# Adamtaranto/frisk

Measured on AMD Instinct MI355X. Metric: windows/sec (k=1..8, w=5kb, s=1kb), higher is better.
Workload: dtype u8/u4 counts + f64 scores

## Files before the change

### frisk_amd/csrc/profile_kernels.h

```cpp
#pragma once
#include "frisk_device.h"

#define FRISK_PROF_NT 1024

struct ProfRange {
    const uint32_t* __restrict__ codes;
    const uint32_t* __restrict__ inv;
    const uint32_t* __restrict__ low;
    int64_t p0, p1;
    int mask_host;
    __device__ int64_t w_first() const { return p0 >> 5; }
    __device__ int64_t w_end() const { return (p1 + 31) >> 5; }
    __device__ void chunk(int64_t i, int64_t chunk_words, int64_t& wb, int64_t& we) const {
        wb = w_first() + i * chunk_words;
        we = wb + chunk_words;
        if (we > w_end()) we = w_end();
    }
};

__device__ __forceinline__ uint32_t topbits(int64_t k) {
    k = k < 0 ? 0 : (k > 32 ? 32 : k);
    return uint32_t(0xFFFFFFFF00000000ull >> k);
}

struct ProfWord {
    uint32_t inr;
    uint32_t other;
    uint64_t V;
    uint64_t NP;
    uint64_t lo64, hi64;
};

__device__ __forceinline__ ProfWord load_word(const ProfRange& r, int64_t wq) {
    const int64_t base = wq << 5;
    const uint32_t i0 = r.inv[wq], i1 = r.inv[wq + 1], l0 = r.low[wq], l1 = r.low[wq + 1];
    const uint32_t c0 = r.codes[2 * wq], c1 = r.codes[2 * wq + 1], c2 = r.codes[2 * wq + 2];
    const uint32_t e0 = i0 | (r.mask_host ? l0 : 0u), e1 = i1 | (r.mask_host ? l1 : 0u);
    ProfWord W;
    W.inr = topbits(r.p1 - base) & ~topbits(r.p0 - base);
    W.other = i0 | l0;
    W.V = ~((uint64_t(e0) << 32) | e1);
    W.NP = ~((uint64_t(i0 & l0) << 32) | (i1 & l1));
    W.lo64 = (uint64_t(c0) << 32) | c1;
    W.hi64 = (uint64_t(c1) << 32) | c2;
    return W;
}

template <bool K8>
__device__ __forceinline__ uint64_t run_starts(uint64_t M, int k) {
    uint64_t F = M;
    if (K8) { F &= F << 1; F &= F << 2; F &= F << 4; }
    else for (int s = 1; s < k; ++s) F &= M << s;
    return F;
}

template <int BITS>
__device__ __forceinline__ uint32_t code_at(const ProfWord& W, int j) {
    return uint32_t((j < 16 ? W.lo64 : W.hi64) >> (64 - BITS - 2 * (j & 15))) & ((1u << BITS) - 1u);
}

template <int BITS>
__device__ __forceinline__ void add_runs(const ProfWord& W, uint32_t todo, int kmin, int kmax, unsigned long long* __restrict__ raw) {
    while (todo) {
        const int j = __clz(int(todo));
        todo &= ~(0x80000000u >> j);
        int run = __clzll((long long)(~(W.V << j)));
        run = run < kmax ? run : kmax;
        if (run >= kmin) atomicAdd(&raw[table_offset(kmin, run) + (code_at<BITS>(W, j) >> (BITS - 2 * run))], 1ull);
    }
}

__device__ __forceinline__ unsigned long long wave_sum(unsigned long long v) {
    for (int o = 32; o > 0; o >>= 1) v += __shfl_down(v, o);
    return v;
}

struct ProfScalars {
    unsigned long long tot = 0, kpos = 0, nn = 0;
    template <bool K8>
    __device__ __forceinline__ void add(const ProfWord& W, int kmax) {
        const uint64_t G = run_starts<K8>(W.NP, kmax);
        const uint32_t real = uint32_t(W.NP >> 32) & W.inr;
        tot += __popc(real);
        nn += __popc(real & W.other);
        kpos += __popc(uint32_t(G >> 32) & W.inr);
    }
    __device__ __forceinline__ void flush(unsigned long long* __restrict__ tail) {
        tot = wave_sum(tot);
        kpos = wave_sum(kpos);
        nn = wave_sum(nn);
        if ((threadIdx.x & 63) == 0) {
            if (tot) atomicAdd(&tail[0], tot);
            if (kpos) atomicAdd(&tail[1], kpos);
            if (nn) atomicAdd(&tail[2], nn);
        }
    }
};

__device__ __forceinline__ void clear_table(uint32_t* hist, uint32_t nwords) {
    for (uint32_t b = threadIdx.x; b < nwords / 4; b += blockDim.x) reinterpret_cast<uint4*>(hist)[b] = make_uint4(0, 0, 0, 0);
    if (nwords < 4) for (uint32_t b = threadIdx.x; b < nwords; b += blockDim.x) hist[b] = 0;
}
__device__ __forceinline__ void flush_table32(const uint32_t* hist, uint32_t nbins, unsigned long long* __restrict__ dst) {
    for (uint32_t b = threadIdx.x; b < nbins; b += blockDim.x) {
        const uint32_t v = hist[b];
        if (v) atomicAdd(&dst[b], (unsigned long long)v);
    }
}

struct HalfTable {
    uint32_t* hist;
    uint32_t nbins, halfbit, mine;
    int shK;
    __device__ __forceinline__ HalfTable(uint32_t* hist_, int kmax, int halves, int half)
        : hist(hist_), nbins((1u << (2 * kmax)) / uint32_t(halves)), halfbit(halves == 2 ? nbins : 0u), mine(half ? halfbit : 0u),
          shK(16 - 2 * kmax) {}
    __device__ __forceinline__ void operator()(uint32_t c16) const {
        const uint32_t code = c16 >> shK;
        if ((code & halfbit) == mine) atomicAdd(&hist[code & (nbins - 1)], 1u);
    }
};

template <bool K8, class Full>
__device__ __forceinline__ unsigned long long walk_words(const ProfRange& r, int64_t wb, int64_t we, int kmin, int kmax, bool rest,
                                                         unsigned long long* __restrict__ raw, int nprof, const Full& full) {
    ProfScalars S;
    unsigned long long counted = 0;
    for (int64_t wq = wb + threadIdx.x; wq < we; wq += blockDim.x) {
        const ProfWord W = load_word(r, wq);
        const uint64_t F = run_starts<K8>(W.V, kmax);
        const uint32_t fullm = uint32_t(F >> 32) & W.inr;
#pragma unroll
        for (int j = 0; j < 32; ++j)
            if (fullm & (0x80000000u >> j)) full(code_at<16>(W, j));
        if (rest) {
            counted += uint32_t(__popc(fullm));
            add_runs<16>(W, uint32_t(W.V >> 32) & ~uint32_t(F >> 32) & W.inr, kmin, kmax, raw);
            S.add<K8>(W, kmax);
        }
    }
    if (rest) S.flush(raw + nprof);
    return counted;
}

__global__ __launch_bounds__(FRISK_PROF_NT) void profile_add_kernel(const uint32_t* __restrict__ codes,
                                                                     const uint32_t* __restrict__ inv,
                                                                     const uint32_t* __restrict__ low, int64_t p0, int64_t p1,
                                                                     int kmin, int kmax, int mask_host, int nprof,
                                                                     int halves, int64_t chunk_words,
                                                                     unsigned long long* __restrict__ raw) {
    extern __shared__ __attribute__((aligned(16))) uint32_t hist[];
    const int half = int(blockIdx.x) % halves;
    const HalfTable table(hist, kmax, halves, half);
    clear_table(hist, table.nbins);
    __syncthreads();
    const ProfRange r{codes, inv, low, p0, p1, mask_host};
    int64_t wb, we;
    r.chunk(int64_t(blockIdx.x) / halves, chunk_words, wb, we);
    walk_words<false>(r, wb, we, kmin, kmax, half == 0, raw, nprof, table);
    __syncthreads();
    flush_table32(hist, table.nbins, raw + table_offset(kmin, kmax) + uint32_t(half) * table.nbins);
}

__global__ __launch_bounds__(FRISK_PROF_NT) void profile_add16_kernel(const uint32_t* __restrict__ codes,
                                                                       const uint32_t* __restrict__ inv,
                                                                       const uint32_t* __restrict__ low, int64_t p0, int64_t p1,
                                                                       int kmin, int mask_host, int nprof, int64_t chunk_words,
                                                                       unsigned long long* __restrict__ raw) {
    constexpr int K = 8;
    constexpr uint32_t NW = (1u << (2 * K)) / 2;
    extern __shared__ __attribute__((aligned(16))) uint32_t hist[];
    __shared__ unsigned long long red[2];
    clear_table(hist, NW);
    if (threadIdx.x < 2) red[threadIdx.x] = 0ull;
    __syncthreads();
    const ProfRange r{codes, inv, low, p0, p1, mask_host};
    int64_t wb, we;
    r.chunk(int64_t(blockIdx.x), chunk_words, wb, we);
    const int64_t offK = table_offset(kmin, K);
    const unsigned long long counted = wave_sum(walk_words<true>(r, wb, we, kmin, K, true, raw, nprof, [&](uint32_t code) {
        atomicAdd(&hist[code >> 1], 1u << ((code & 1u) * 16u));
    }));
    if ((threadIdx.x & 63) == 0 && counted) atomicAdd(&red[0], counted);
    __syncthreads();
    {
        unsigned long long sum = 0;
        for (uint32_t b = threadIdx.x; b < NW; b += blockDim.x) { const uint32_t v = hist[b]; sum += (v & 0xFFFFu) + (v >> 16); }
        sum = wave_sum(sum);
        if ((threadIdx.x & 63) == 0 && sum) atomicAdd(&red[1], sum);
    }
    __syncthreads();
    if (red[0] == red[1]) {
        for (uint32_t b = threadIdx.x; b < NW; b += blockDim.x) {
            const uint32_t v = hist[b];
            if (v & 0xFFFFu) atomicAdd(&raw[offK + 2u * b], (unsigned long long)(v & 0xFFFFu));
            if (v >> 16) atomicAdd(&raw[offK + 2u * b + 1u], (unsigned long long)(v >> 16));
        }
        return;
    }
    for (int half = 0; half < 2; ++half) {
        __syncthreads();
        clear_table(hist, NW);
        __syncthreads();
        walk_words<true>(r, wb, we, kmin, K, false, raw, nprof, HalfTable(hist, K, 2, half));
        __syncthreads();
        flush_table32(hist, NW, raw + offK + uint32_t(half) * NW);
    }
}

__global__ __launch_bounds__(256) void profile_add_big_kernel(const uint32_t* __restrict__ codes, const uint32_t* __restrict__ inv,
                                                               const uint32_t* __restrict__ low, int64_t p0, int64_t p1, int kmin,
                                                               int kmax, int mask_host, int nprof,
                                                               unsigned long long* __restrict__ raw) {
    const ProfRange r{codes, inv, low, p0, p1, mask_host};
    ProfScalars S;
    for (int64_t wq = r.w_first() + int64_t(blockIdx.x) * blockDim.x + threadIdx.x; wq < r.w_end(); wq += int64_t(gridDim.x) * blockDim.x) {
        const ProfWord W = load_word(r, wq);
        add_runs<24>(W, uint32_t(W.V >> 32) & W.inr, kmin, kmax, raw);
        S.add<false>(W, kmax);
    }
    S.flush(raw + nprof);
}

__global__ __launch_bounds__(256) void marginalize_kernel(int64_t* __restrict__ cnt, int kmin, int x) {
    const int64_t q = int64_t(blockIdx.x) * blockDim.x + threadIdx.x;
    if (q >= (int64_t(1) << (2 * x))) return;
    const int64_t* up = cnt + table_offset(kmin, x + 1) + 4 * q;
    cnt[table_offset(kmin, x) + q] += up[0] + up[1] + up[2] + up[3];
}

__global__ __launch_bounds__(1024) void marginalize_low_kernel(int64_t* __restrict__ cnt, int kmin, int x_hi) {
    for (int x = x_hi; x >= kmin; --x) {
        const int64_t n = int64_t(1) << (2 * x);
        int64_t* dst = cnt + table_offset(kmin, x);
        const int64_t* up = cnt + table_offset(kmin, x + 1);
        for (int64_t q = threadIdx.x; q < n; q += blockDim.x) dst[q] += up[4 * q] + up[4 * q + 1] + up[4 * q + 2] + up[4 * q + 3];
        __threadfence_block();
        __syncthreads();
    }
}

__global__ __launch_bounds__(256) void symmetrize_kernel(const int64_t* __restrict__ fwd, int64_t* __restrict__ sym,
                                                          int kmin, int kmax) {
    const int64_t t = int64_t(blockIdx.x) * blockDim.x + threadIdx.x;
    for (int x = kmin; x <= kmax; ++x) {
        const int64_t off = table_offset(kmin, x), n = int64_t(1) << (2 * x);
        if (t >= off && t < off + n) {
            const uint32_t c = uint32_t(t - off);
            sym[t] = fwd[t] + fwd[off + revcomp_code(c, x)];
        }
    }
}

#pragma clang fp contract(off)
__global__ __launch_bounds__(1024) void profile_meta_kernel(const int64_t* __restrict__ cnt, const int64_t* __restrict__ raw_tail,
                                                             int kmin, int kmax, int64_t* __restrict__ meta) {
    __shared__ long long part[16];
    const int64_t n = int64_t(1) << (2 * kmax);
    const int64_t* top = cnt + table_offset(kmin, kmax);
    long long s = 0;
    for (int64_t i = threadIdx.x; i < n; i += blockDim.x) s += top[i];
    for (int o = 32; o > 0; o >>= 1) s += __shfl_down(s, o);
    if ((threadIdx.x & 63) == 0) part[threadIdx.x >> 6] = s;
    __syncthreads();
    if (threadIdx.x == 0) {
        long long counted = 0;
        for (int w = 0; w < int(blockDim.x >> 6); ++w) counted += part[w];
        meta[0] = raw_tail[0];
        meta[1] = raw_tail[1] - counted;
        meta[2] = raw_tail[2];
    }
}

__global__ __launch_bounds__(256) void genome_ivom_kernel(const int64_t* __restrict__ sym, int kmin, int kmax,
                                                           const int64_t* __restrict__ meta, double* __restrict__ ig) {
    const int64_t k = int64_t(blockIdx.x) * blockDim.x + threadIdx.x;
    if (k >= (int64_t(1) << (2 * kmax))) return;
    const int64_t genome_space = meta[0] - meta[2];
    unsigned long long W = 0;
    double I = 0.0;
    bool bad = false;
    for (int x = kmin; x <= kmax; ++x) {
        const int64_t c = sym[table_offset(kmin, x) + (k >> (2 * (kmax - x)))];
        const unsigned long long wt = (unsigned long long)c << (2 * x);
        W += wt;
        const int64_t D = (genome_space - (x - 1)) * 2;
        if (W == 0 || D == 0) { bad = true; break; }
        const double p = double(c) / double(D);
        const double a = double(wt) / double(W);
        I = (x == kmin) ? a * p : a * p + ((1.0 - a) * I);
    }
    ig[k] = bad ? __longlong_as_double(0x7FF8000000000000LL) : I;
}
```

Before: 68.18 million.

## Repack k=8 shared histogram by top bit and add all-full wave fast path

Changes the packed 16-bit shared histogram so the top code bit picks the upper or lower half-word instead of the lowest bit. The index becomes a plain shift-and-mask of the unmasked code window, and the half select uses a bitfield extract. It also adds a wave-uniform fast path: when every lane's word is fully covered by k-runs, the per-j bit tests and the add_runs loop are skipped. The flush maps the two half-words to the bins b and NW+b. This adds inline asm and a wave vote, and correctness depends on the new index mapping matching the raw table layout.

```diff
diff --git a/frisk_amd/csrc/profile_kernels.h b/frisk_amd/csrc/profile_kernels.h
--- a/frisk_amd/csrc/profile_kernels.h
+++ b/frisk_amd/csrc/profile_kernels.h
@@ -1,5 +1,8 @@
 #pragma once
 #include "frisk_device.h"
+#ifdef FRISK_PROFILE_DEBUG
+#include <cassert>
+#endif
 
 #define FRISK_PROF_NT 1024
 
@@ -59,6 +62,10 @@
     return uint32_t((j < 16 ? W.lo64 : W.hi64) >> (64 - BITS - 2 * (j & 15))) & ((1u << BITS) - 1u);
 }
 
+__device__ __forceinline__ uint32_t code4_at(const ProfWord& W, int j) {
+    return uint32_t((j < 16 ? W.lo64 : W.hi64) >> (46 - 2 * (j & 15)));
+}
+
 template <int BITS>
 __device__ __forceinline__ void add_runs(const ProfWord& W, uint32_t todo, int kmin, int kmax, unsigned long long* __restrict__ raw) {
     while (todo) {
@@ -115,8 +122,8 @@
     __device__ __forceinline__ HalfTable(uint32_t* hist_, int kmax, int halves, int half)
         : hist(hist_), nbins((1u << (2 * kmax)) / uint32_t(halves)), halfbit(halves == 2 ? nbins : 0u), mine(half ? halfbit : 0u),
           shK(16 - 2 * kmax) {}
-    __device__ __forceinline__ void operator()(uint32_t c16) const {
-        const uint32_t code = c16 >> shK;
+    __device__ __forceinline__ void operator()(uint32_t c4) const {
+        const uint32_t code = ((c4 >> 2) & 0xFFFFu) >> shK;
         if ((code & halfbit) == mine) atomicAdd(&hist[code & (nbins - 1)], 1u);
     }
 };
@@ -130,9 +137,21 @@
         const ProfWord W = load_word(r, wq);
         const uint64_t F = run_starts<K8>(W.V, kmax);
         const uint32_t fullm = uint32_t(F >> 32) & W.inr;
+        if (__all(fullm == 0xFFFFFFFFu)) {
+#pragma unroll
+            for (int j = 0; j < 32; ++j) full(code4_at(W, j));
+            if (rest) {
+#ifdef FRISK_PROFILE_DEBUG
+                assert((uint32_t(W.V >> 32) & ~uint32_t(F >> 32) & W.inr) == 0u);
+#endif
+                counted += 32u;
+                S.add<K8>(W, kmax);
+            }
+            continue;
+        }
 #pragma unroll
         for (int j = 0; j < 32; ++j)
-            if (fullm & (0x80000000u >> j)) full(code_at<16>(W, j));
+            if (fullm & (0x80000000u >> j)) full(code4_at(W, j));
         if (rest) {
             counted += uint32_t(__popc(fullm));
             add_runs<16>(W, uint32_t(W.V >> 32) & ~uint32_t(F >> 32) & W.inr, kmin, kmax, raw);
@@ -178,8 +197,10 @@
     int64_t wb, we;
     r.chunk(int64_t(blockIdx.x), chunk_words, wb, we);
     const int64_t offK = table_offset(kmin, K);
-    const unsigned long long counted = wave_sum(walk_words<true>(r, wb, we, kmin, K, true, raw, nprof, [&](uint32_t code) {
-        atomicAdd(&hist[code >> 1], 1u << ((code & 1u) * 16u));
+    const unsigned long long counted = wave_sum(walk_words<true>(r, wb, we, kmin, K, true, raw, nprof, [&](uint32_t c4) {
+        uint32_t top;
+        asm("v_bfe_u32 %0, %1, 17, 1" : "=v"(top) : "v"(c4));
+        atomicAdd(&hist[(c4 >> 2) & (NW - 1u)], __umul24(top, 0xFFFFu) + 1u);
     }));
     if ((threadIdx.x & 63) == 0 && counted) atomicAdd(&red[0], counted);
     __syncthreads();
@@ -193,8 +214,8 @@
     if (red[0] == red[1]) {
         for (uint32_t b = threadIdx.x; b < NW; b += blockDim.x) {
             const uint32_t v = hist[b];
-            if (v & 0xFFFFu) atomicAdd(&raw[offK + 2u * b], (unsigned long long)(v & 0xFFFFu));
-            if (v >> 16) atomicAdd(&raw[offK + 2u * b + 1u], (unsigned long long)(v >> 16));
+            if (v & 0xFFFFu) atomicAdd(&raw[offK + b], (unsigned long long)(v & 0xFFFFu));
+            if (v >> 16) atomicAdd(&raw[offK + NW + b], (unsigned long long)(v >> 16));
         }
         return;
     }
```

Measured after the change: 68.85 million, median of 6. No clear change (+1.0%).
